# Jason9339/Wavelet-Noise-in-ray-tracing

Measured on AMD Instinct MI355X. Metric: Mnoise-samples/sec (3D wavelet, octave=4), higher is better.
Workload: dtype f32; 1 GPU; 512^3 dense 3D WNoise grid, tile=128, octave=4 (configs[1]); tile=128, seed=12345, octave=4, device=AMD Radeon Graphics (gfx950:sramecc+:xnack-)

## Files before the change

wavelet-noise-in-ray-tracing_amd/csrc/wn_api.hip:

```cpp
#include "wn_internal.hpp"

#include <algorithm>
#include <cstdlib>
#include <cstring>
#include <map>
#include <mutex>
#include <numeric>
#include <random>
#include <utility>
#include <vector>

namespace wn {

static char g_private_rand_state[256];
static std::mutex g_rand_mu;
static int g_rand_depth = 0;
static char *g_rand_caller = nullptr;

RandStateGuard::RandStateGuard()
{
    std::lock_guard<std::mutex> lock(g_rand_mu);
    if (g_rand_depth++ == 0) {
        static bool initialised = false;
        if (!initialised) {
// ... 295 lines not shown
    if (e != hipSuccess) {
        delete x;
        return hip_fail(e, "hipEventCreate");
    }
    *t = x;
    return WN_OK;
}
int wn_timer_start(wn_timer *t, void *stream)
{
    WN_ENTRY();
    if (!t) return fail(WN_ERR_INVALID, "timer is NULL");
    WN_HIP(hipEventRecord(t->start, as_stream(stream)));
    return WN_OK;
}
int wn_timer_stop(wn_timer *t, void *stream)
{
    WN_ENTRY();
    if (!t) return fail(WN_ERR_INVALID, "timer is NULL");
    WN_HIP(hipEventRecord(t->stop, as_stream(stream)));
    return WN_OK;
}
int wn_timer_elapsed_ms(wn_timer *t, float *ms)
{
    WN_ENTRY();
    if (!t || !ms) return fail(WN_ERR_INVALID, "timer/ms is NULL");
    WN_HIP(hipEventSynchronize(t->stop));
    WN_HIP(hipEventElapsedTime(ms, t->start, t->stop));
    return WN_OK;
}
void wn_timer_destroy(wn_timer *t)
{
    WN_ENTRY();
    if (!t) return;
    if (t->start) (void)hipEventDestroy(t->start);
    if (t->stop) (void)hipEventDestroy(t->stop);
    delete t;
}

int wn_gaussian_fill(uint32_t seed, size_t count, float *out_host)
{
    WN_ENTRY();
    if (count && !out_host) return fail(WN_ERR_INVALID, "out_host is NULL");
    std::mt19937 engine(seed);
    std::normal_distribution<float> gauss(0.0f, 1.0f);
    for (size_t i = 0; i < count; ++i) out_host[i] = gauss(engine);
    return WN_OK;
}

int wn_perlin_permutation(uint32_t seed, int out512_host[512])
{
    WN_ENTRY();
    if (!out512_host) return fail(WN_ERR_INVALID, "out512_host is NULL");
    std::vector<int> v(256);
    std::iota(v.begin(), v.end(), 0);
    std::shuffle(v.begin(), v.end(), std::mt19937(seed));
    for (int i = 0; i < 256; ++i) out512_host[i] = out512_host[i + 256] = v[i];
    return WN_OK;
}

int wn_tile_even_size(int requested) { return (requested % 2 != 0) ? requested + 1 : requested; }

static int tile_alloc(int n, int dims, wn_tile **out)
{
    if (!out) return fail(WN_ERR_INVALID, "out is NULL");
    *out = nullptr;
    if (dims != 2 && dims != 3) return fail(WN_ERR_INVALID, "dims must be 2 or 3 (got %d)", dims);
    if (n < 0) return fail(WN_ERR_INVALID, "tile size must be >= 0 (got %d)", n);
    if (n > 1024 || (dims == 3 && n > 1024)) return fail(WN_ERR_INVALID, "tile size %d too large", n);
    int rc = require_device();
    if (rc) return rc;
    wn_tile *t = new wn_tile();
    t->n = n;
    t->dims = dims;
    t->count = (dims == 2) ? (size_t)n * n : (size_t)n * n * n;
    (void)hipGetDevice(&t->device);
    if (t->count) {
        hipError_t e = hipMalloc(reinterpret_cast<void **>(&t->dev), t->count * sizeof(float));
        if (e != hipSuccess) {
            delete t;
            hip_fail(e, "hipMalloc(tile)");
            return WN_ERR_ALLOC;
        }
    }
    *out = t;
    return WN_OK;
}

int wn_tile_create(int n, int dims, const float *coeffs_host, wn_tile **out)
{
    WN_ENTRY();
    if (!coeffs_host) n = 0;
    if (n % 2 != 0)
        return fail(WN_ERR_INVALID, "wn_tile_create: coefficient tiles have even size (got %d)", n);
    int rc = tile_alloc(n, dims, out);
    if (rc) return rc;
    if ((*out)->count) {
        hipError_t e = hipMemcpy((*out)->dev, coeffs_host, (*out)->count * sizeof(float),
                                 hipMemcpyHostToDevice);
        if (e != hipSuccess) {
            wn_tile_destroy(*out);
            *out = nullptr;
            return hip_fail(e, "hipMemcpy(tile)");
        }
        rc = tile_build_padded(*out, nullptr);
        if (rc) {
            wn_tile_destroy(*out);
            *out = nullptr;
            return rc;
        }
    }
    return WN_OK;
}

int wn_tile_generate_from_field(int n, int dims, const float *field_host, wn_tile **out)
{
    WN_ENTRY();
    if (!field_host && n > 0) return fail(WN_ERR_INVALID, "field_host is NULL");
    if (n % 2 != 0) return fail(WN_ERR_INVALID, "tile size must be even (got %d)", n);
    int rc = tile_alloc(n, dims, out);
    if (rc) return rc;
    wn_tile *t = *out;
    if (!t->count) return WN_OK;
    float *field_dev = nullptr;
    hipError_t e = hipMalloc(reinterpret_cast<void **>(&field_dev), t->count * sizeof(float));
    if (e == hipSuccess)
        e = hipMemcpy(field_dev, field_host, t->count * sizeof(float), hipMemcpyHostToDevice);
    if (e != hipSuccess) {
        if (field_dev) (void)hipFree(field_dev);
        wn_tile_destroy(t);
        *out = nullptr;
        return hip_fail(e, "tile field upload");
    }
    rc = wn::tilegen_filter(t, field_dev, nullptr);
    hipError_t se = hipStreamSynchronize(nullptr);
    (void)hipFree(field_dev);
    if (rc == WN_OK && se != hipSuccess) rc = hip_fail(se, "tile generation");
    if (rc == WN_OK) rc = tile_build_padded(t, nullptr);
    if (rc) {
        wn_tile_destroy(t);
        *out = nullptr;
    }
    return rc;
}

int wn_tile_generate(int n, int dims, uint32_t seed, wn_tile **out)
{
    WN_ENTRY();
    if (n < 0) return fail(WN_ERR_INVALID, "tile size must be >= 0");
    if (dims != 2 && dims != 3) return fail(WN_ERR_INVALID, "dims must be 2 or 3 (got %d)", dims);
    const int even = wn_tile_even_size(n);
    if (even != n)
        fprintf(stderr, "Warning: Tile size adjusted to %d (must be even)\n", even);
    const size_t count = (dims == 2) ? (size_t)even * even : (size_t)even * even * even;
    std::vector<float> field(count);
    wn_gaussian_fill(seed, count, field.data());
    return wn_tile_generate_from_field(even, dims, field.data(), out);
}

int wn_tile_size(const wn_tile *t) { return t ? t->n : 0; }
int wn_tile_dims(const wn_tile *t) { return t ? t->dims : 0; }
size_t wn_tile_count(const wn_tile *t) { return t ? t->count : 0; }
const float *wn_tile_device_ptr(const wn_tile *t) { return t ? t->dev : nullptr; }

int wn_tile_download(const wn_tile *t, float *out_host)
{
    WN_ENTRY();
    if (!t) return fail(WN_ERR_INVALID, "tile is NULL");
    if (!t->count) return WN_OK;
    if (!out_host) return fail(WN_ERR_INVALID, "out_host is NULL");
    WN_HIP(hipMemcpy(out_host, t->dev, t->count * sizeof(float), hipMemcpyDeviceToHost));
    return WN_OK;
}

void wn_tile_destroy(wn_tile *t)
{
    WN_ENTRY();
    if (!t) return;
    if (t->dev) (void)hipFree(t->dev);
    if (t->dev_padded) (void)hipFree(t->dev_padded);
    delete t;
}

int wn_perm_create(const int table512_host[512], wn_perm **out)
{
    WN_ENTRY();
    if (!out) return fail(WN_ERR_INVALID, "out is NULL");
    *out = nullptr;
    if (!table512_host) return fail(WN_ERR_INVALID, "table is NULL");
    uint8_t bytes[512];
    for (int i = 0; i < 512; ++i) {
        if (table512_host[i] < 0 || table512_host[i] > 255)
            return fail(WN_ERR_INVALID, "permutation entry %d out of 0..255", i);
        bytes[i] = (uint8_t)table512_host[i];
    }
    int rc = require_device();
    if (rc) return rc;
    wn_perm *p = new wn_perm();
    std::memcpy(p->host, table512_host, sizeof(p->host));
    (void)hipGetDevice(&p->device);
    hipError_t e = hipMalloc(reinterpret_cast<void **>(&p->dev), 512);
    if (e == hipSuccess) e = hipMemcpy(p->dev, bytes, 512, hipMemcpyHostToDevice);
    if (e != hipSuccess) {
        if (p->dev) (void)hipFree(p->dev);
        delete p;
        return hip_fail(e, "perm upload");
    }
    *out = p;
    return WN_OK;
}

int wn_perm_create_seeded(uint32_t seed, wn_perm **out)
{
    WN_ENTRY();
    int table[512];
    wn_perlin_permutation(seed, table);
    return wn_perm_create(table, out);
}

int wn_perm_download(const wn_perm *p, int out512_host[512])
{
    WN_ENTRY();
    if (!p || !out512_host) return fail(WN_ERR_INVALID, "perm/out is NULL");
    uint8_t bytes[512];
    WN_HIP(hipMemcpy(bytes, p->dev, 512, hipMemcpyDeviceToHost));
    for (int i = 0; i < 512; ++i) out512_host[i] = bytes[i];
    return WN_OK;
}

void wn_perm_destroy(wn_perm *p)
{
    WN_ENTRY();
    if (!p) return;
    if (p->dev) (void)hipFree(p->dev);
    delete p;
}

}
```

wavelet-noise-in-ray-tracing_amd/csrc/wn_internal.hpp:

```cpp
#pragma once

#include <hip/hip_runtime.h>

#include <cmath>
#include <cstdarg>
#include <cstddef>
#include <cstdint>
#include <cstdio>

#include "wn_eval.hpp"
#include "wnoise.h"
#include "wnoise_advect.h"

typedef float v4f __attribute__((ext_vector_type(4)));

struct wn_tile {
    int n = 0;
    int dims = 0;
    size_t count = 0;
    float *dev = nullptr;
    float *dev_padded = nullptr;
    int device = 0;
};

struct wn_perm {
    int host[512];
    uint8_t *dev = nullptr;
    int device = 0;
};

struct wn_timer {
    hipEvent_t start = nullptr, stop = nullptr;
};

namespace wn {

void set_error(const char *fmt, ...);
int fail(int code, const char *fmt, ...);
int hip_fail(hipError_t e, const char *what);
int require_device();

inline hipStream_t as_stream(void *s) { return reinterpret_cast<hipStream_t>(s); }

class RandStateGuard {
  public:
    RandStateGuard();
    ~RandStateGuard();
    RandStateGuard(const RandStateGuard &) = delete;
    RandStateGuard &operator=(const RandStateGuard &) = delete;
};
#define WN_ENTRY() ::wn::RandStateGuard wn_rand_state_guard_

#define WN_HIP(call)                                            \
    do {                                                        \
        hipError_t _e = (call);                                 \
        if (_e != hipSuccess) return ::wn::hip_fail(_e, #call); \
    } while (0)

#define WN_LAUNCH_CHECK(name)                                    \
    do {                                                         \
        hipError_t _e = hipGetLastError();                       \
        if (_e != hipSuccess) return ::wn::hip_fail(_e, name);   \
    } while (0)

struct GridArgs {
    int den, nx, ny, z0, nz;
    float base_range, octave_scale, post_scale;
    int z_const_mode;
    float z_const;
    float out_scale;
};

int check_grid(const wn_grid *g, bool needs_z, GridArgs *out);

inline float inv_den_of(int den) { return ((den & (den - 1)) == 0) ? 1.0f / (float)den : 0.0f; }

int current_device();
int device_compute_units(int dev);
bool ensure_dynamic_lds(const void *kernel, int dev, size_t bytes);
int check_handle_device(int handle_device, const char *what);
int check_tile(const wn_tile *tile, int dims, const char *entry);
int check_perm(const wn_perm *perm, const char *entry);

inline bool vec4_ok(const float *out, int nx) { return nx % 4 == 0 && (reinterpret_cast<uintptr_t>(out) & 15) == 0; }

constexpr size_t kStrideBlockCap = 256u * 8u * 8u;
inline int stride_blocks(size_t total, size_t cap = kStrideBlockCap)
{
    const size_t b = (total + 255) / 256;
    return (int)(b < 1 ? 1 : (b > cap ? cap : b));
}

struct LatticeStep {
    double step;
    double pmax;
    double slack;
    long long extent(int samples) const { return (long long)floor((samples - 1) * step + slack) + 1 + 3; }
    bool two_mids() const { return 3.0 * step + slack <= 1.0; }
};

inline bool lattice_step(const GridArgs &g, float oscale, bool with_z_const, bool signed_step, double margin_cells,
                         LatticeStep *ls)
{
    double step = (double)g.base_range * (double)oscale * (double)g.post_scale / g.den;
// ... 148 lines not shown
```

wavelet-noise-in-ray-tracing_amd/csrc/wn_wavelet_multiband.hip:

```cpp
#include "wn_internal.hpp"

#include <algorithm>
#include <cmath>
#include <type_traits>

namespace {

using wn::GridArgs;

typedef float v4f __attribute__((ext_vector_type(4)));
typedef float v2f __attribute__((ext_vector_type(2)));

constexpr int kMaxNB = 5;
constexpr int kWW = 8, kPW = 4, kSW = 4;
constexpr int kWaves = kWW + kPW + kSW;
constexpr int kPasses = 2 * kPW;
constexpr int kBX = 512, kBY = 8, kBZ = 8;
constexpr int kRing = 4;
constexpr int kSlotZ = 8, kSlotX = 16;
constexpr int kMaxK = 5;
constexpr int kRRow = kPasses * 64;
constexpr int kRPlane = kBY * kRRow;
constexpr int kRingFloats = kRing * kBY * kBX;
constexpr int kBoxFloats = 6144;
constexpr int kDmaPlanes = kMaxNB;
constexpr int kDmaLanded = kBZ - 2;

struct MbBand {
    float oscale;
    float factor;
    int first_pass;
    int K;
    int box_off;
    int rowlen;
};

struct MbArgs {
    const float *coef;
    float *out;
    int n, nmask;
    GridArgs g;
    float inv_den;
    int nbx, nby, nbz;
    int all_full;
    MbBand band[kMaxNB];
    int pass_band[kPasses];
};

__device__ __forceinline__ float readlane_f(float v, int l)
{
    return __int_as_float(__builtin_amdgcn_readlane(__float_as_int(v), l));
}

template <int NB>
__global__ __launch_bounds__(64 * kWaves) void grid3d_mbp_kernel(const MbArgs a)
{
    extern __shared__ __attribute__((aligned(16))) float lds[];
    __shared__ __attribute__((aligned(16))) float s_box[kBoxFloats];
    __shared__ int s_mid[3][NB][32];
    __shared__ float s_w[3][NB][kSlotX][3];
    __shared__ float s_oscale[NB];
    __shared__ __attribute__((aligned(16))) float s_wy[NB][kMaxK][kBY];
    __shared__ float s_wz[NB][64];
    __shared__ int s_prep[NB][4];
    __shared__ int s_bandc[NB][4];

    const int tid = threadIdx.x, lane = tid & 63;
    const int wave = __builtin_amdgcn_readfirstlane(tid >> 6);
    const bool is_window = wave < kWW, is_collapse = wave >= kWW && wave < kWW + kPW;
    const GridArgs &g = a.g;
    float *const ring = lds + 2 * kRPlane;

    const int nyz = a.nby * a.nbz;
    const long long total = (long long)a.nbx * nyz;
    const int item0 = (int)(total * blockIdx.x / gridDim.x), item1 = (int)(total * (blockIdx.x + 1) / gridDim.x);
    const int nb = item1 - item0;
    if (nb <= 0) return;
    const int G = nb * kBZ;

    struct Brick { int bx, by, bz; };
    auto brick_of = [&](int item) {
        Brick k;
        k.bx = item / nyz;
        k.by = (item - k.bx * nyz) / a.nbz;
        k.bz = item - k.bx * nyz - k.by * a.nbz;
        return k;
    };
    auto advance = [&](Brick &k) {
        if (++k.bz == a.nbz) { k.bz = 0; ++k.by; }
        if (k.by == a.nby) { k.by = 0; ++k.bx; }
    };

    auto fill_tables = [&](int buf, const Brick &k) {
        int tt = tid;
        asm volatile("" : "+v"(tt));
        const int b = tt >> 5, slot = tt & 31;
        if (b < NB && slot < kSlotX + 2) {
            int idx;
            if (slot < kSlotZ) idx = min(k.by * kBY + slot, g.ny - 1);
            else if (slot < kSlotX) idx = g.z0 + min(k.bz * kBZ + slot - kSlotZ, g.nz - 1);
            else idx = (slot == kSlotX) ? k.bx * kBX : min(k.bx * kBX + kBX - 1, g.nx - 1);
            const float c = wn::lattice_coord_fast(idx, (float)g.den, a.inv_den, g.base_range, s_oscale[b], g.post_scale);
            int m;
            float w0, w1, w2;
            wn::bspline(c, m, w0, w1, w2);
            s_mid[buf][b][slot] = m;
            if (slot < kSlotX) {
                s_w[buf][b][slot][0] = w0;
                s_w[buf][b][slot][1] = w1;
                s_w[buf][b][slot][2] = w2;
            }
        }
    };
    auto sgpr = [](int v) { return __builtin_amdgcn_readfirstlane(v); };
    auto fresh_rows = [&](int b, int K, int tA, int tB, bool same_column) {
        const int d = sgpr(s_mid[tB][b][kSlotZ]) - sgpr(s_mid[tA][b][kSlotZ]);
        return (same_column && d >= 0 && d <= 2) ? d : K;
    };

    auto derive_tables = [&](int b, int tA, int tB, bool same_column, bool first) {
        const int l = lane;
        {
            const int K = s_bandc[b][0];
            const int kz0 = s_mid[tB][b][kSlotZ] - 1;
            const int kzm = (K == 4) ? (kz0 & 3) : ((kz0 + 20 * 65536) % 5);
            {
                const int zi = l >> 3, j = l & 7;
                int t0 = kzm + (s_mid[tB][b][kSlotZ + zi] - s_mid[tB][b][kSlotZ]);
                t0 -= (t0 >= K) ? K : 0;
                const float w0 = s_w[tB][b][kSlotZ + zi][0], w1 = s_w[tB][b][kSlotZ + zi][1], w2 = s_w[tB][b][kSlotZ + zi][2];
                s_wz[b][l] = j == 0 ? w0 : j == 1 ? w1 : j == 2 ? w2 : __int_as_float(t0);
            }
            if (l < kMaxK * kBY) {
                const int j = l >> 3, yi = l & 7;
                const int dd = j - (s_mid[tB][b][yi] - s_mid[tB][b][0]);
                const float w0 = s_w[tB][b][yi][0], w1 = s_w[tB][b][yi][1], w2 = s_w[tB][b][yi][2];
                float f = a.band[0].factor;
#pragma unroll
                for (int bb = 1; bb < NB; ++bb) f = (b == bb) ? a.band[bb].factor : f;
                s_wy[b][j][yi] = ((unsigned)dd <= 2u ? (dd == 0 ? w0 : dd == 1 ? w1 : w2) : 0.0f) * f;
            }
            if (l == 0) {
                const int dz = s_mid[tB][b][kSlotZ] - s_mid[tA][b][kSlotZ];
                s_prep[b][0] = kzm;
                s_prep[b][1] = (!first && same_column && dz >= 0 && dz <= 2) ? dz : K;
                s_prep[b][2] = (s_mid[tB][b][kSlotX] - 1) & 3;
            }
        }
    };

    Brick cur = brick_of(item0), nxt = cur;
    advance(nxt);
    Brick nxt2 = nxt;
    advance(nxt2);
    if (tid < NB) {
        int K = a.band[0].K, box_off = a.band[0].box_off, rowlen = a.band[0].rowlen, fp = a.band[0].first_pass;
#pragma unroll
        for (int bb = 1; bb < NB; ++bb) {
            K = (tid == bb) ? a.band[bb].K : K;
            box_off = (tid == bb) ? a.band[bb].box_off : box_off;
            rowlen = (tid == bb) ? a.band[bb].rowlen : rowlen;
            fp = (tid == bb) ? a.band[bb].first_pass : fp;
        }
        s_bandc[tid][0] = K;
        s_bandc[tid][1] = box_off;
        s_bandc[tid][2] = rowlen;
        s_bandc[tid][3] = fp;
        float os = a.band[0].oscale;
#pragma unroll
        for (int bb = 1; bb < NB; ++bb) os = (tid == bb) ? a.band[bb].oscale : os;
        s_oscale[tid] = os;
    }
    __syncthreads();
    fill_tables(0, cur);
    if (nb > 1) fill_tables(1, nxt);
    __syncthreads();
    int tb = 0, t = 0;
    auto next_brick = [&]() {
        cur = nxt;
        nxt = nxt2;
        advance(nxt2);
        tb = (tb == 2) ? 0 : tb + 1;
        ++t;
    };

// ... 48 lines not shown
        };
        auto p1_slice = [&](float *Rw, int zi, const auto &yc, float wzv, auto kc) {
            constexpr int K = decltype(kc)::value;
            if constexpr (K > 0) {
                const float w0 = readlane_f(wzv, zi * 8), w1 = readlane_f(wzv, zi * 8 + 1), w2 = readlane_f(wzv, zi * 8 + 2);
                const int t0 = __builtin_amdgcn_readlane(__float_as_int(wzv), zi * 8 + 3);
                auto taps = [&](auto tc) {
                    constexpr int T0 = decltype(tc)::value, T1 = (T0 + 1) % K, T2 = (T0 + 2) % K;
#pragma unroll
                    for (int p2 = 0; p2 < kBY / 2; ++p2) {
                        v2f v = v2f{w0, w0} * yc[p2][T0];
                        v = __builtin_elementwise_fma(v2f{w1, w1}, yc[p2][T1], v);
                        v = __builtin_elementwise_fma(v2f{w2, w2}, yc[p2][T2], v);
                        Rw[(2 * p2) * kRRow] = v.x;
                        Rw[(2 * p2 + 1) * kRRow] = v.y;
                    }
                };
                using std::integral_constant;
                if (t0 == 0) taps(integral_constant<int, 0>{});
                else if (t0 == 1) taps(integral_constant<int, 1>{});
                else if (t0 == 2) taps(integral_constant<int, 2>{});
                else if (t0 == 3 || K == 4) taps(integral_constant<int, 3>{});
                else taps(integral_constant<int, K - 1>{});
            }
        };
        auto collapse_role = [&](auto k0c, auto k1c) {
            constexpr int K0 = decltype(k0c)::value, K1 = decltype(k1c)::value;
            v2f yc0[kBY / 2][K0 > 0 ? K0 : 1], yc1[kBY / 2][K1 > 0 ? K1 : 1];
            float wzv0 = 0.0f, wzv1 = 0.0f;
            float *const Rw0 = lds + 64 * ps[0].id + lane, *const Rw1 = lds + 64 * ps[1].id + lane;
            wn::lds_barrier();
            prep_brick(ps[0], yc0, wzv0, k0c);
            prep_brick(ps[1], yc1, wzv1, k1c);
            p1_slice(Rw0, 0, yc0, wzv0, k0c);
            p1_slice(Rw1, 0, yc1, wzv1, k1c);
            wn::lds_barrier();
            for (int gp = 0; gp < G + 2; ++gp) {
                const int zi = gp & (kBZ - 1);
                if (gp < G) {
                    if (gp + 1 < G) {
                        if (zi == kBZ - 1) {
                            prep_brick(ps[0], yc0, wzv0, k0c);
                            prep_brick(ps[1], yc1, wzv1, k1c);
                        }
                        const int rs = ((gp + 1) & 1) * kRPlane;
                        p1_slice(Rw0 + rs, (gp + 1) & (kBZ - 1), yc0, wzv0, k0c);
                        p1_slice(Rw1 + rs, (gp + 1) & (kBZ - 1), yc1, wzv1, k1c);
                    }
                    if (zi == kBZ - 1) next_brick();
                }
                wn::lds_barrier();
            }
        };
        using std::integral_constant;
        const int k0 = pk[0], k1 = pk[1];
        if (k0 == 4 && k1 == 4) collapse_role(integral_constant<int, 4>{}, integral_constant<int, 4>{});
        else if (k0 == 4 && k1 == 5) collapse_role(integral_constant<int, 4>{}, integral_constant<int, 5>{});
        else if (k0 == 5 && k1 == 4) collapse_role(integral_constant<int, 5>{}, integral_constant<int, 4>{});
        else if (k0 == 5 && k1 == 5) collapse_role(integral_constant<int, 5>{}, integral_constant<int, 5>{});
        else if (k0 == 4) collapse_role(integral_constant<int, 4>{}, integral_constant<int, 0>{});
        else if (k0 == 5) collapse_role(integral_constant<int, 5>{}, integral_constant<int, 0>{});
        else collapse_role(integral_constant<int, 0>{}, integral_constant<int, 0>{});
    } else if (is_window) {
        const int xw = (wave >> 2) & 1, wr = wave & 3;
        float ww[NB][4][4];
        int wbase[NB];
        auto x_weights = [&](int tbuf, int bx) {
            const float den = (float)g.den;
            const int x0 = bx * kBX + xw * 256 + lane * 4;
            float xbase[4];
#pragma unroll
            for (int q = 0; q < 4; ++q) {
                const float xi = (float)min(x0 + q, g.nx - 1);
                xbase[q] = ((a.inv_den != 0.0f) ? xi * a.inv_den : xi / den) * g.base_range;
            }
#pragma unroll
            for (int b = 0; b < NB; ++b) {
                int m[4];
                float w[4][3];
#pragma unroll
                for (int q = 0; q < 4; ++q) {
                    float cc = xbase[q] * a.band[b].oscale;
                    cc = cc * g.post_scale;
                    wn::bspline(cc, m[q], w[q][0], w[q][1], w[q][2]);
                }
                wbase[b] = 64 * a.band[b].first_pass + m[0] - s_mid[tbuf][b][kSlotX];
#pragma unroll
                for (int q = 0; q < 4; ++q) {
                    const bool up = m[q] != m[0];
                    ww[b][q][0] = up ? 0.0f : w[q][0];
                    ww[b][q][1] = up ? w[q][0] : w[q][1];
                    ww[b][q][2] = up ? w[q][1] : w[q][2];
                    ww[b][q][3] = up ? w[q][2] : 0.0f;
                }
            }
        };
        auto phaseC = [&](int rslot, int ringslot) {
            float acc[2][4];
            const float *Rp = lds + rslot * kRPlane + wr * kRRow;
#pragma unroll
            for (int b = 0; b < NB; ++b) {
                float v[2][4];
#pragma unroll
                for (int h = 0; h < 2; ++h)
#pragma unroll
                    for (int i = 0; i < 4; ++i) v[h][i] = Rp[h * 4 * kRRow + wbase[b] + i];
#pragma unroll
                for (int h = 0; h < 2; ++h)
#pragma unroll
                    for (int q = 0; q < 4; ++q) {
                        float s = (b == 0) ? ww[b][q][0] * v[h][0] : __builtin_fmaf(ww[b][q][0], v[h][0], acc[h][q]);
                        s = __builtin_fmaf(ww[b][q][1], v[h][1], s);
                        s = __builtin_fmaf(ww[b][q][2], v[h][2], s);
                        s = __builtin_fmaf(ww[b][q][3], v[h][3], s);
                        acc[h][q] = s;
                    }
            }
#pragma unroll
            for (int h = 0; h < 2; ++h)
                *reinterpret_cast<v4f *>(ring + (ringslot * kBY + wr + 4 * h) * kBX + xw * 256 + lane * 4) =
                    v4f{acc[h][0], acc[h][1], acc[h][2], acc[h][3]};
        };

        x_weights(0, cur.bx);
        wn::lds_barrier();
        wn::lds_barrier();
        for (int gp = 0; gp < G + 2; ++gp) {
            const int zi = gp & (kBZ - 1);
            if (gp < G) {
                phaseC(gp & 1, gp & (kRing - 1));
                if (zi == kBZ - 1) {
                    const int tb1 = (tb == 2) ? 0 : tb + 1, tb2 = (tb1 == 2) ? 0 : tb1 + 1;
                    if (t + 2 < nb) fill_tables(tb2, nxt2);
                    if (t + 1 < nb && nxt.bx != cur.bx) x_weights(tb1, nxt.bx);
                    next_brick();
                }
            }
            wn::lds_barrier();
        }
    } else {
        const int sw = wave - (kWW + kPW);
        int bK[NB], bBox[NB], bRow[NB];
#pragma unroll
        for (int b = 0; b < NB; ++b) {
            bK[b] = sgpr(s_bandc[b][0]);
            bBox[b] = sgpr(s_bandc[b][1]);
            bRow[b] = sgpr(s_bandc[b][2]);
        }
        auto request_band = [&](auto bc, int tA, int tB, bool same_column, bool first) {
            constexpr int b = decltype(bc)::value;
            if constexpr (b < NB) {
                const int K = bK[b];
                const int d = first ? K : fresh_rows(b, K, tA, tB, same_column);
                const int jy0 = sgpr(s_mid[tB][b][0]) - 1, kz0 = sgpr(s_mid[tB][b][kSlotZ]) - 1 + (K - d);
                const int r = min(lane, K * K - 1);
                const int f = (K == 4) ? (r >> 2) : ((r * 13) >> 6);
                const int j = r - f * K;
                const int rowoff = (((kz0 + f) & a.nmask) * a.n + ((jy0 + j) & a.nmask)) * a.n;
                const int ix0 = (sgpr(s_mid[tB][b][kSlotX]) - 1) & ~3;
                const unsigned voff = (unsigned)((ix0 + 4 * lane) & a.nmask) * 4u;
                for (int rr = sw; rr < d * K; rr += kSW) {
                    const char *rowp = reinterpret_cast<const char *>(a.coef + __builtin_amdgcn_readlane(rowoff, rr));
                    if (4 * lane < bRow[b])
                        __builtin_amdgcn_global_load_lds((const __attribute__((address_space(1))) void *)(rowp + voff),
                                                         (__attribute__((address_space(3))) void *)&s_box[bBox[b] + rr * bRow[b]],
                                                         16, 0, 0);
                }
            }
        };
        Brick sb = cur;
        const size_t plane_stride = (size_t)g.ny * g.nx;
        float *orow = nullptr;
        auto brick_pointer = [&]() {
            orow = a.out + ((size_t)(sb.bz * kBZ) * g.ny + sb.by * kBY + 2 * sw) * g.nx + sb.bx * kBX + lane * 4;
        };
        brick_pointer();
        auto store_plane = [&](int p) {
            const int zi = p & (kBZ - 1), ringslot = p & (kRing - 1);
            const float *src = ring + (ringslot * kBY + 2 * sw) * kBX + lane * 4;
            v4f v[4];
#pragma unroll
            for (int q = 0; q < 4; ++q) v[q] = *reinterpret_cast<const v4f *>(src + (q >> 1) * kBX + (q & 1) * 256);
            if (a.all_full) {
#pragma unroll
                for (int q = 0; q < 4; ++q) *reinterpret_cast<v4f *>(orow + (size_t)(q >> 1) * g.nx + (q & 1) * 256) = v[q];
            } else {
                const int z = sb.bz * kBZ + zi;
#pragma unroll
                for (int q = 0; q < 4; ++q) {
                    const int row = 2 * sw + (q >> 1), xh = q & 1;
                    const int y = sb.by * kBY + row, x = sb.bx * kBX + xh * 256 + lane * 4;
                    if (y < g.ny && z < g.nz && x + 3 < g.nx)
                        *reinterpret_cast<v4f *>(orow + (size_t)(q >> 1) * g.nx + (q & 1) * 256) = v[q];
                }
            }
            orow += plane_stride;
            if (zi == kBZ - 1) {
                advance(sb);
                brick_pointer();
            }
        };

        using std::integral_constant;
        request_band(integral_constant<int, 0>{}, 0, 0, false, true);
        request_band(integral_constant<int, 1>{}, 0, 0, false, true);
        request_band(integral_constant<int, 2>{}, 0, 0, false, true);
        request_band(integral_constant<int, 3>{}, 0, 0, false, true);
        request_band(integral_constant<int, 4>{}, 0, 0, false, true);
        for (int b = sw; b < NB; b += kSW) derive_tables(b, 0, 0, false, true);
        asm volatile("s_waitcnt vmcnt(0)" ::: "memory");
        wn::lds_barrier();
        wn::lds_barrier();
        for (int gp = 0; gp < G + 2; ++gp) {
            const int zi = gp & (kBZ - 1);
            if (gp >= 2) store_plane(gp - 2);
            if (gp < G) {
                if (zi < NB && t + 1 < nb) {
                    const int tb1 = (tb == 2) ? 0 : tb + 1;
                    const bool same = nxt.bx == cur.bx && nxt.by == cur.by;
                    if (zi == 0) request_band(integral_constant<int, 0>{}, tb, tb1, same, false);
                    else if (zi == 1) request_band(integral_constant<int, 1>{}, tb, tb1, same, false);
                    else if (zi == 2) request_band(integral_constant<int, 2>{}, tb, tb1, same, false);
                    else if (zi == 3) request_band(integral_constant<int, 3>{}, tb, tb1, same, false);
                    else request_band(integral_constant<int, 4>{}, tb, tb1, same, false);
                }
                if (zi == kBZ - 2 && t + 1 < nb)
                    for (int b = sw; b < NB; b += kSW)
                        derive_tables(b, tb, (tb == 2) ? 0 : tb + 1, nxt.bx == cur.bx && nxt.by == cur.by, false);
                if (zi == kDmaLanded) {
                    if (a.all_full) asm volatile("s_waitcnt vmcnt(%0)" ::"n"(4 * (kDmaLanded - kDmaPlanes + 1)) : "memory");
                    else asm volatile("s_waitcnt vmcnt(0)" ::: "memory");
                }
                if (zi == kBZ - 1) next_brick();
            }
            wn::lds_barrier();
        }
    }
}

template <int NB>
bool launch_mbp(const MbArgs &a, size_t lds, long long bricks, hipStream_t s)
{
    const void *fn = reinterpret_cast<const void *>(&grid3d_mbp_kernel<NB>);
    if (!wn::ensure_dynamic_lds(fn, wn::current_device(), lds)) return false;
    const int cus = wn::device_compute_units(wn::current_device());
    const int grid = (int)std::min<long long>(bricks, cus);
    hipLaunchKernelGGL((grid3d_mbp_kernel<NB>), dim3(grid), dim3(64 * kWaves), lds, s, a);
    return true;
}

}

namespace wn {

int multiband_try(const wn_tile *tile, const GridArgs &g, int nbands, const float *oscale, const float *weights,
                  float out_div, float *out_dev, hipStream_t stream, int min_bricks_per_cu)
{
    if (nbands < 1 || nbands > kMaxNB || tile->n == 0 || wn::pow2_mask(tile->n) < 0) return kDeclined;
    if (g.nx <= 256 || !vec4_ok(out_dev, g.nx) || g.ny <= 0 || g.nz <= 0 || g.z_const_mode || g.z0 < 0) return kDeclined;
    MbArgs a{};
    int passes = 0, box_off = 0;
    for (int w = 0; w < kPasses; ++w) a.pass_band[w] = -1;
    for (int b = 0; b < nbands; ++b) {
        LatticeStep ls;
        if (!lattice_step(g, oscale[b], false, false, 0.0, &ls) || !ls.two_mids()) return kDeclined;
        const int K = (int)std::max<long long>(4, std::max(ls.extent(kBY), ls.extent(kBZ)));
        if (K > kMaxK) return kDeclined;
        const int ex = (int)ls.extent(kBX) + 1;
        const int np = (ex + 63) / 64;
        if (passes + np > kPasses) return kDeclined;
        a.band[b].first_pass = passes;
        for (int p = 0; p < np; ++p) a.pass_band[passes++] = b;
        a.band[b].oscale = oscale[b];
        a.band[b].factor = (float)((double)(weights ? weights[b] : 1.0f) * (double)g.out_scale / (double)out_div);
        a.band[b].K = K;
        a.band[b].rowlen = (ex + 3 + 3) & ~3;
        if (a.band[b].rowlen > 256) return kDeclined;
        a.band[b].box_off = box_off;
        box_off += K * K * a.band[b].rowlen;
    }
    if (box_off > kBoxFloats) return kDeclined;
    const size_t lds = (size_t)(2 * kRPlane + kRingFloats) * sizeof(float);
    a.coef = tile->dev;
    a.out = out_dev;
    a.n = tile->n;
    a.nmask = wn::pow2_mask(tile->n);
    a.g = g;
    a.inv_den = wn::inv_den_of(g.den);
    a.nbx = (g.nx + kBX - 1) / kBX;
    a.nby = (g.ny + kBY - 1) / kBY;
    a.nbz = (g.nz + kBZ - 1) / kBZ;
    a.all_full = (g.nx % kBX == 0 && g.ny % kBY == 0 && g.nz % kBZ == 0) ? 1 : 0;
    const long long bricks = (long long)a.nbx * a.nby * a.nbz;
    if (bricks > 0x7fffffffLL / kBZ) return kDeclined;
    if (bricks < (long long)min_bricks_per_cu * wn::device_compute_units(wn::current_device())) return kDeclined;
    if ((long long)a.nbx * kBX * 10 > (long long)g.nx * 11) return kDeclined;
    bool ok;
    switch (nbands) {
    case 1: ok = launch_mbp<1>(a, lds, bricks, stream); break;
    case 2: ok = launch_mbp<2>(a, lds, bricks, stream); break;
    case 3: ok = launch_mbp<3>(a, lds, bricks, stream); break;
    case 4: ok = launch_mbp<4>(a, lds, bricks, stream); break;
    default: ok = launch_mbp<5>(a, lds, bricks, stream); break;
    }
    if (!ok) return kDeclined;
    WN_LAUNCH_CHECK("grid3d_mbp_kernel");
    return WN_OK;
}

}
```

Before: 1.389 million Msamples/s.

## Merge lower octave bands into one pre-upsampled coefficient box before evaluation

For three or more bands whose scales double each step, a new prepass kernel algebraically folds all lower octaves into a single dense coefficient field sampled at the top band's lattice (half-cell shifted). It uses B-spline upsampling weights of 0.75/0.25 and writes the field to per-tile scratch. The main kernel then evaluates only two spline bands instead of NB, reading the merged box from scratch. The volume is processed in z-chunks sized to fit the scratch. The cost is an extra kernel launch per chunk, scratch memory traffic, and an event to order reuse of the scratch buffer.

Result: slower. 1.368 million Msamples/s (-1.5%).

```diff
diff --git a/wavelet-noise-in-ray-tracing_amd/csrc/wn_api.hip b/wavelet-noise-in-ray-tracing_amd/csrc/wn_api.hip
--- a/wavelet-noise-in-ray-tracing_amd/csrc/wn_api.hip
+++ b/wavelet-noise-in-ray-tracing_amd/csrc/wn_api.hip
@@ -401,6 +401,15 @@
             return WN_ERR_ALLOC;
         }
     }
+    if (t->count && dims == 3) {
+        hipError_t e = hipMalloc(reinterpret_cast<void **>(&t->merge_scratch), wn::kMergeScratchBytes);
+        if (e == hipSuccess) e = hipEventCreateWithFlags(&t->merge_done, hipEventDisableTiming);
+        if (e != hipSuccess) {
+            wn_tile_destroy(t);
+            hip_fail(e, "hipMalloc(tile scratch)");
+            return WN_ERR_ALLOC;
+        }
+    }
     *out = t;
     return WN_OK;
 }
@@ -497,6 +506,8 @@
     if (!t) return;
     if (t->dev) (void)hipFree(t->dev);
     if (t->dev_padded) (void)hipFree(t->dev_padded);
+    if (t->merge_scratch) (void)hipFree(t->merge_scratch);
+    if (t->merge_done) (void)hipEventDestroy(t->merge_done);
     delete t;
 }
 
diff --git a/wavelet-noise-in-ray-tracing_amd/csrc/wn_internal.hpp b/wavelet-noise-in-ray-tracing_amd/csrc/wn_internal.hpp
--- a/wavelet-noise-in-ray-tracing_amd/csrc/wn_internal.hpp
+++ b/wavelet-noise-in-ray-tracing_amd/csrc/wn_internal.hpp
@@ -9,6 +9,7 @@
 #include <cstdio>
 
 #include "wn_eval.hpp"
+#include "wn_merge_plan.hpp"
 #include "wnoise.h"
 #include "wnoise_advect.h"
 
@@ -20,6 +21,8 @@
     size_t count = 0;
     float *dev = nullptr;
     float *dev_padded = nullptr;
+    float *merge_scratch = nullptr;
+    hipEvent_t merge_done = nullptr;
     int device = 0;
 };
 
diff --git a/wavelet-noise-in-ray-tracing_amd/csrc/wn_merge_plan.hpp b/wavelet-noise-in-ray-tracing_amd/csrc/wn_merge_plan.hpp
--- /dev/null
+++ b/wavelet-noise-in-ray-tracing_amd/csrc/wn_merge_plan.hpp
@@ -0,0 +1,74 @@
+#pragma once
+
+#include <algorithm>
+#include <climits>
+#include <cmath>
+#include <cstddef>
+
+namespace wn {
+
+constexpr size_t kMergeScratchBytes = (size_t)16 << 20;
+constexpr int kMergeBrickX = 512, kMergeBrickYZ = 8;
+
+struct MergeRange {
+    long long lo, hi;
+    long long count() const { return hi - lo + 1; }
+};
+
+inline long long merge_mid_min(double step, double slack, long long i) { return (long long)ceil(i * step - 1.0 - slack); }
+inline long long merge_mid_max(double step, double slack, long long i) { return (long long)ceil(i * step - 1.0 + slack); }
+
+inline long long merge_floor4(long long v) { return v - (((v % 4) + 4) % 4); }
+
+inline MergeRange merge_rows(double step, double slack, long long i0, long long count, int K)
+{
+    const long long last = i0 + count - 1, last_brick = i0 + (count - 1) / kMergeBrickYZ * kMergeBrickYZ;
+    MergeRange r;
+    r.lo = merge_mid_min(step, slack, i0) - 1;
+    r.lo -= ((r.lo % 2) + 2) % 2;
+    r.hi = std::max(merge_mid_max(step, slack, last) + 1, merge_mid_max(step, slack, last_brick) - 1 + (K - 1));
+    return r;
+}
+
+inline MergeRange merge_columns(double step, double slack, long long nx, int rowlen)
+{
+    const long long last_brick = (nx - 1) / kMergeBrickX * kMergeBrickX;
+    MergeRange r;
+    r.lo = merge_floor4(merge_mid_min(step, slack, 0) - 1);
+    const long long end = std::max(merge_mid_max(step, slack, nx - 1) + 2, merge_floor4(merge_mid_max(step, slack, last_brick) - 1) + rowlen);
+    r.hi = r.lo + ((end - r.lo + 3) / 4) * 4 - 1;
+    return r;
+}
+
+inline long long merge_z_rows_bound(double step, double slack, long long planes, int K)
+{
+    const long long last_brick = (planes - 1) / kMergeBrickYZ * kMergeBrickYZ;
+    const long long by_last = (long long)floor((planes - 1) * step + 2.0 * slack) + 1 + 2;
+    const long long by_brick = (long long)floor(last_brick * step + 2.0 * slack) + 1 + (K - 1);
+    return std::max(by_last, by_brick) + 1 + 1;
+}
+
+struct MergePlan {
+    MergeRange x, y;
+    long long z_rows;
+    long long chunk_planes;
+};
+
+inline bool merge_plan(double step, double slack, int nx, int ny, int K, int rowlen, size_t capacity, MergePlan *p)
+{
+    if (nx <= 0 || ny <= 0 || !(step >= 0.0)) return false;
+    p->x = merge_columns(step, slack, nx, rowlen);
+    p->y = merge_rows(step, slack, 0, ny, K);
+    const long long footprint = p->x.count() * p->y.count();
+    if (footprint <= 0 || (unsigned long long)footprint > capacity) return false;
+    p->z_rows = (long long)(capacity / (unsigned long long)footprint);
+    if (merge_z_rows_bound(step, slack, kMergeBrickYZ, K) > p->z_rows) return false;
+    long long planes = (long long)(INT_MAX / kMergeBrickYZ) * kMergeBrickYZ;
+    if (step > 0.0 && (double)p->z_rows / step < (double)planes - 2 * kMergeBrickYZ)
+        planes = (long long)((double)p->z_rows / step) / kMergeBrickYZ * kMergeBrickYZ + kMergeBrickYZ;
+    while (planes > kMergeBrickYZ && merge_z_rows_bound(step, slack, planes, K) > p->z_rows) planes -= kMergeBrickYZ;
+    p->chunk_planes = planes;
+    return true;
+}
+
+}
diff --git a/wavelet-noise-in-ray-tracing_amd/csrc/wn_wavelet_multiband.hip b/wavelet-noise-in-ray-tracing_amd/csrc/wn_wavelet_multiband.hip
--- a/wavelet-noise-in-ray-tracing_amd/csrc/wn_wavelet_multiband.hip
+++ b/wavelet-noise-in-ray-tracing_amd/csrc/wn_wavelet_multiband.hip
@@ -23,6 +23,9 @@
 constexpr int kRPlane = kBY * kRRow;
 constexpr int kRingFloats = kRing * kBY * kBX;
 constexpr int kBoxFloats = 6144;
+constexpr int kBoxFloatsMerged = 8192;
+constexpr int kMergeFrom = 3;
+constexpr int box_floats(int nb) { return nb >= kMergeFrom ? kBoxFloatsMerged : kBoxFloats; }
 constexpr int kDmaPlanes = kMaxNB;
 constexpr int kDmaLanded = kBZ - 2;
 
@@ -45,18 +48,25 @@
     int all_full;
     MbBand band[kMaxNB];
     int pass_band[kPasses];
+    const float *msrc;
+    int m_ox, m_oy, m_oz, m_sx, m_sy, m_sz;
 };
+
+template <int NB>
+constexpr bool from_merged_box(int b) { return NB >= kMergeFrom && b == 0; }
 
 __device__ __forceinline__ float readlane_f(float v, int l)
 {
     return __int_as_float(__builtin_amdgcn_readlane(__float_as_int(v), l));
 }
 
-template <int NB>
+template <int NBANDS>
 __global__ __launch_bounds__(64 * kWaves) void grid3d_mbp_kernel(const MbArgs a)
 {
+    constexpr bool kMerged = NBANDS >= kMergeFrom;
+    constexpr int NB = kMerged ? 2 : NBANDS;
     extern __shared__ __attribute__((aligned(16))) float lds[];
-    __shared__ __attribute__((aligned(16))) float s_box[kBoxFloats];
+    __shared__ __attribute__((aligned(16))) float s_box[box_floats(NBANDS)];
     __shared__ int s_mid[3][NB][32];
     __shared__ float s_w[3][NB][kSlotX][3];
     __shared__ float s_oscale[NB];
@@ -100,7 +110,8 @@
             if (slot < kSlotZ) idx = min(k.by * kBY + slot, g.ny - 1);
             else if (slot < kSlotX) idx = g.z0 + min(k.bz * kBZ + slot - kSlotZ, g.nz - 1);
             else idx = (slot == kSlotX) ? k.bx * kBX : min(k.bx * kBX + kBX - 1, g.nx - 1);
-            const float c = wn::lattice_coord_fast(idx, (float)g.den, a.inv_den, g.base_range, s_oscale[b], g.post_scale);
+            float c = wn::lattice_coord_fast(idx, (float)g.den, a.inv_den, g.base_range, s_oscale[b], g.post_scale);
+            if constexpr (kMerged) c = (b == 0) ? c - 0.5f : c;
             int m;
             float w0, w1, w2;
             wn::bspline(c, m, w0, w1, w2);
@@ -315,6 +326,7 @@
                 for (int q = 0; q < 4; ++q) {
                     float cc = xbase[q] * a.band[b].oscale;
                     cc = cc * g.post_scale;
+                    if constexpr (kMerged) cc = (b == 0) ? cc - 0.5f : cc;
                     wn::bspline(cc, m[q], w[q][0], w[q][1], w[q][2]);
                 }
                 wbase[b] = 64 * a.band[b].first_pass + m[0] - s_mid[tbuf][b][kSlotX];
@@ -389,11 +401,22 @@
                 const int r = min(lane, K * K - 1);
                 const int f = (K == 4) ? (r >> 2) : ((r * 13) >> 6);
                 const int j = r - f * K;
-                const int rowoff = (((kz0 + f) & a.nmask) * a.n + ((jy0 + j) & a.nmask)) * a.n;
                 const int ix0 = (sgpr(s_mid[tB][b][kSlotX]) - 1) & ~3;
-                const unsigned voff = (unsigned)((ix0 + 4 * lane) & a.nmask) * 4u;
+                int rowoff;
+                unsigned voff;
+                const float *src;
+                if constexpr (from_merged_box<NBANDS>(b)) {
+                    const int kr = min(max(kz0 + f - a.m_oz, 0), a.m_sz - 1), jr = min(max(jy0 + j - a.m_oy, 0), a.m_sy - 1);
+                    rowoff = (kr * a.m_sy + jr) * a.m_sx + min(max(ix0 - a.m_ox, 0), a.m_sx - bRow[b]);
+                    voff = (unsigned)(4 * lane) * 4u;
+                    src = a.msrc;
+                } else {
+                    rowoff = (((kz0 + f) & a.nmask) * a.n + ((jy0 + j) & a.nmask)) * a.n;
+                    voff = (unsigned)((ix0 + 4 * lane) & a.nmask) * 4u;
+                    src = a.coef;
+                }
                 for (int rr = sw; rr < d * K; rr += kSW) {
-                    const char *rowp = reinterpret_cast<const char *>(a.coef + __builtin_amdgcn_readlane(rowoff, rr));
+                    const char *rowp = reinterpret_cast<const char *>(src + __builtin_amdgcn_readlane(rowoff, rr));
                     if (4 * lane < bRow[b])
                         __builtin_amdgcn_global_load_lds((const __attribute__((address_space(1))) void *)(rowp + voff),
                                                          (__attribute__((address_space(3))) void *)&s_box[bBox[b] + rr * bRow[b]],
@@ -471,6 +494,189 @@
     }
 }
 
+constexpr int kMgX = 32, kMgY = 8, kMgZ = 8;
+constexpr int kMgLds = 7 * 7 * 18;
+constexpr int kMgC = 6 * 6 * 17;
+
+struct MergeArgs {
+    const float *coef;
+    float *M;
+    int n, nmask;
+    int ox, oy, oz, sx, sy, sz;
+    float factor[kMaxNB - 1];
+};
+
+struct MgRegion {
+    const float *p;
+    int x0, y0, z0, nx, ny;
+};
+
+template <bool FIRST>
+__device__ __forceinline__ float merge_value(float f, int hx, int hy, int hz, const MgRegion &c, const MgRegion &prev)
+{
+    const int ex = hx & 1, ey = hy & 1, ez = hz & 1;
+    const int mx = hx >> 1, my = hy >> 1, mz = hz >> 1;
+    const float wx[2] = {ex ? 0.25f : 0.75f, ex ? 0.75f : 0.25f}, wy[2] = {ey ? 0.25f : 0.75f, ey ? 0.75f : 0.25f},
+                wz[2] = {ez ? 0.25f : 0.75f, ez ? 0.75f : 0.25f};
+    float w[2][2][2];
+#pragma unroll
+    for (int dz = 0; dz < 2; ++dz)
+#pragma unroll
+        for (int dy = 0; dy < 2; ++dy)
+#pragma unroll
+            for (int dx = 0; dx < 2; ++dx) w[dz][dy][dx] = (wz[dz] * wy[dy]) * wx[dx];
+    const float *cp = c.p + ((mz - c.z0) * c.ny + (my - c.y0)) * c.nx + (mx - c.x0);
+    float cs = 0.0f;
+#pragma unroll
+    for (int dz = 0; dz < 2; ++dz)
+#pragma unroll
+        for (int dy = 0; dy < 2; ++dy)
+#pragma unroll
+            for (int dx = 0; dx < 2; ++dx) {
+                const float v = cp[(dz * c.ny + dy) * c.nx + dx];
+                cs = (dz + dy + dx == 0) ? w[dz][dy][dx] * v : __builtin_fmaf(w[dz][dy][dx], v, cs);
+            }
+    if constexpr (FIRST) {
+        return f * cs;
+    } else {
+        const float *p = prev.p + ((mz - 1 + ez - prev.z0) * prev.ny + (my - 1 + ey - prev.y0)) * prev.nx + (mx - 1 + ex - prev.x0);
+        float hs = 0.0f;
+#pragma unroll
+        for (int dz = 0; dz < 2; ++dz)
+#pragma unroll
+            for (int dy = 0; dy < 2; ++dy)
+#pragma unroll
+                for (int dx = 0; dx < 2; ++dx) {
+                    const float v = p[(dz * prev.ny + dy) * prev.nx + dx];
+                    hs = (dz + dy + dx == 0) ? w[1 - dz][1 - dy][1 - dx] * v : __builtin_fmaf(w[1 - dz][1 - dy][1 - dx], v, hs);
+                }
+        return __builtin_fmaf(f, cs, hs);
+    }
+}
+
+__device__ __forceinline__ int mg_div(int e, int inv) { return (e * inv) >> 18; }
+__device__ __forceinline__ int mg_inv(int d) { return ((1 << 18) + d - 1) / d; }
+
+__device__ __forceinline__ void merge_group(float f, const float (&cv)[2][2][2], const float (&qv)[3][3][3], float (&out)[2][2][2])
+{
+#pragma unroll
+    for (int oz = 0; oz < 2; ++oz)
+#pragma unroll
+        for (int oy = 0; oy < 2; ++oy)
+#pragma unroll
+            for (int ox = 0; ox < 2; ++ox) {
+                float cs = 0.0f, hs = 0.0f;
+#pragma unroll
+                for (int dz = 0; dz < 2; ++dz)
+#pragma unroll
+                    for (int dy = 0; dy < 2; ++dy)
+#pragma unroll
+                        for (int dx = 0; dx < 2; ++dx) {
+                            const float wd = ((dz == oz ? 0.75f : 0.25f) * (dy == oy ? 0.75f : 0.25f)) * (dx == ox ? 0.75f : 0.25f);
+                            const float we = ((dz != oz ? 0.75f : 0.25f) * (dy != oy ? 0.75f : 0.25f)) * (dx != ox ? 0.75f : 0.25f);
+                            const float q = qv[oz + dz][oy + dy][ox + dx];
+                            cs = (dz + dy + dx == 0) ? wd * cv[dz][dy][dx] : __builtin_fmaf(wd, cv[dz][dy][dx], cs);
+                            hs = (dz + dy + dx == 0) ? we * q : __builtin_fmaf(we, q, hs);
+                        }
+                out[oz][oy][ox] = __builtin_fmaf(f, cs, hs);
+            }
+}
+
+template <int L>
+__global__ __launch_bounds__(256) void band_merge_kernel(const MergeArgs a)
+{
+    static_assert(L >= 2 && L < kMaxNB, "the bands below the top one of 3..5");
+    __shared__ float s_lvl[2][kMgLds];
+    __shared__ float s_c[L][kMgC];
+    const int tid = threadIdx.x;
+    int lo[L + 1][3], len[L + 1][3];
+    lo[L][0] = a.ox + kMgX * blockIdx.x, len[L][0] = min(kMgX, a.sx - kMgX * (int)blockIdx.x);
+    lo[L][1] = a.oy + kMgY * blockIdx.y, len[L][1] = min(kMgY, a.sy - kMgY * (int)blockIdx.y);
+    lo[L][2] = a.oz + kMgZ * blockIdx.z, len[L][2] = min(kMgZ, a.sz - kMgZ * (int)blockIdx.z);
+#pragma unroll
+    for (int l = L - 1; l >= 1; --l)
+#pragma unroll
+        for (int d = 0; d < 3; ++d) {
+            lo[l][d] = (lo[l + 1][d] >> 1) - 1;
+            len[l][d] = ((lo[l + 1][d] + len[l + 1][d] - 1) >> 1) + 1 - lo[l][d] + 1;
+        }
+    MgRegion c[L + 1];
+    int ccount[L + 1];
+    float cval[L + 1][2];
+    int cix[L + 1], ciy[L + 1];
+    auto c_index = [&](int l, int e) {
+        const int r = mg_div(e, cix[l]), x = e - r * c[l].nx, z = mg_div(r, ciy[l]), y = r - z * c[l].ny;
+        return (((c[l].z0 + z) & a.nmask) * a.n + ((c[l].y0 + y) & a.nmask)) * a.n + ((c[l].x0 + x) & a.nmask);
+    };
+#pragma unroll
+    for (int l = 1; l <= L; ++l) {
+        c[l] = MgRegion{s_c[l - 1], lo[l][0] >> 1, lo[l][1] >> 1, lo[l][2] >> 1, 0, 0};
+        c[l].nx = ((lo[l][0] + len[l][0] - 1) >> 1) + 2 - c[l].x0;
+        c[l].ny = ((lo[l][1] + len[l][1] - 1) >> 1) + 2 - c[l].y0;
+        ccount[l] = c[l].nx * c[l].ny * (((lo[l][2] + len[l][2] - 1) >> 1) + 2 - c[l].z0);
+        cix[l] = mg_inv(c[l].nx), ciy[l] = mg_inv(c[l].ny);
+#pragma unroll
+        for (int k = 0; k < 2; ++k) cval[l][k] = (tid + 256 * k < ccount[l]) ? a.coef[c_index(l, tid + 256 * k)] : 0.0f;
+    }
+#pragma unroll
+    for (int l = 1; l <= L; ++l) {
+#pragma unroll
+        for (int k = 0; k < 2; ++k)
+            if (tid + 256 * k < ccount[l]) s_c[l - 1][tid + 256 * k] = cval[l][k];
+        for (int e = tid + 512; e < ccount[l]; e += 256) s_c[l - 1][e] = a.coef[c_index(l, e)];
+    }
+    __syncthreads();
+#pragma unroll
+    for (int l = 1; l < L; ++l) {
+        const MgRegion prev{s_lvl[(l - 1) & 1], lo[l > 1 ? l - 1 : 1][0], lo[l > 1 ? l - 1 : 1][1], lo[l > 1 ? l - 1 : 1][2],
+                            len[l > 1 ? l - 1 : 1][0], len[l > 1 ? l - 1 : 1][1]};
+        float *cur = s_lvl[l & 1];
+        const int ix = mg_inv(len[l][0]), iy = mg_inv(len[l][1]);
+        for (int e = tid; e < len[l][0] * len[l][1] * len[l][2]; e += 256) {
+            const int r = mg_div(e, ix), x = e - r * len[l][0], z = mg_div(r, iy), y = r - z * len[l][1];
+            const int hx = lo[l][0] + x, hy = lo[l][1] + y, hz = lo[l][2] + z;
+            cur[e] = (l == 1) ? merge_value<true>(a.factor[0], hx, hy, hz, c[l], prev) : merge_value<false>(a.factor[l - 1], hx, hy, hz, c[l], prev);
+        }
+        __syncthreads();
+    }
+    const int gx = tid & 15, gy = (tid >> 4) & 3, gz = tid >> 6;
+    if (2 * gx < len[L][0] && 2 * gy < len[L][1] && 2 * gz < len[L][2]) {
+        const MgRegion &cc = c[L];
+        const MgRegion prev{s_lvl[(L - 1) & 1], lo[L - 1][0], lo[L - 1][1], lo[L - 1][2], len[L - 1][0], len[L - 1][1]};
+        const int jx = (lo[L][0] >> 1) + gx, jy = (lo[L][1] >> 1) + gy, jz = (lo[L][2] >> 1) + gz;
+        float cv[2][2][2], qv[3][3][3], out[2][2][2];
+        const float *cp = cc.p + ((jz - cc.z0) * cc.ny + (jy - cc.y0)) * cc.nx + (jx - cc.x0);
+        const float *qp = prev.p + ((jz - 1 - prev.z0) * prev.ny + (jy - 1 - prev.y0)) * prev.nx + (jx - 1 - prev.x0);
+#pragma unroll
+        for (int dz = 0; dz < 2; ++dz)
+#pragma unroll
+            for (int dy = 0; dy < 2; ++dy)
+#pragma unroll
+                for (int dx = 0; dx < 2; ++dx) cv[dz][dy][dx] = cp[(dz * cc.ny + dy) * cc.nx + dx];
+#pragma unroll
+        for (int dz = 0; dz < 3; ++dz)
+#pragma unroll
+            for (int dy = 0; dy < 3; ++dy)
+#pragma unroll
+                for (int dx = 0; dx < 3; ++dx) qv[dz][dy][dx] = qp[(dz * prev.ny + dy) * prev.nx + dx];
+        merge_group(a.factor[L - 1], cv, qv, out);
+        float *o = a.M + ((size_t)(kMgZ * blockIdx.z + 2 * gz) * a.sy + (kMgY * blockIdx.y + 2 * gy)) * a.sx + (kMgX * blockIdx.x + 2 * gx);
+#pragma unroll
+        for (int oz = 0; oz < 2; ++oz)
+#pragma unroll
+            for (int oy = 0; oy < 2; ++oy)
+                if (2 * gz + oz < len[L][2] && 2 * gy + oy < len[L][1])
+                    *reinterpret_cast<v2f *>(o + ((size_t)oz * a.sy + oy) * a.sx) = v2f{out[oz][oy][0], out[oz][oy][1]};
+    }
+}
+
+template <int L>
+void launch_merge(const MergeArgs &a, hipStream_t s)
+{
+    const dim3 grid((a.sx + kMgX - 1) / kMgX, (a.sy + kMgY - 1) / kMgY, (a.sz + kMgZ - 1) / kMgZ);
+    hipLaunchKernelGGL((band_merge_kernel<L>), grid, dim3(256), 0, s, a);
+}
+
 template <int NB>
 bool launch_mbp(const MbArgs &a, size_t lds, long long bricks, hipStream_t s)
 {
@@ -494,25 +700,53 @@
     MbArgs a{};
     int passes = 0, box_off = 0;
     for (int w = 0; w < kPasses; ++w) a.pass_band[w] = -1;
-    for (int b = 0; b < nbands; ++b) {
-        LatticeStep ls;
-        if (!lattice_step(g, oscale[b], false, false, 0.0, &ls) || !ls.two_mids()) return kDeclined;
-        const int K = (int)std::max<long long>(4, std::max(ls.extent(kBY), ls.extent(kBZ)));
-        if (K > kMaxK) return kDeclined;
-        const int ex = (int)ls.extent(kBX) + 1;
+    auto plan_spline = [&](int s, float os, float factor, LatticeStep *ls) {
+        if (!lattice_step(g, os, false, false, 0.0, ls) || !ls->two_mids()) return false;
+        const int K = (int)std::max<long long>(4, std::max(ls->extent(kBY), ls->extent(kBZ)));
+        if (K > kMaxK) return false;
+        const int ex = (int)ls->extent(kBX) + 1;
         const int np = (ex + 63) / 64;
-        if (passes + np > kPasses) return kDeclined;
-        a.band[b].first_pass = passes;
-        for (int p = 0; p < np; ++p) a.pass_band[passes++] = b;
-        a.band[b].oscale = oscale[b];
-        a.band[b].factor = (float)((double)(weights ? weights[b] : 1.0f) * (double)g.out_scale / (double)out_div);
-        a.band[b].K = K;
-        a.band[b].rowlen = (ex + 3 + 3) & ~3;
-        if (a.band[b].rowlen > 256) return kDeclined;
-        a.band[b].box_off = box_off;
-        box_off += K * K * a.band[b].rowlen;
-    }
+        if (passes + np > kPasses) return false;
+        a.band[s].first_pass = passes;
+        for (int p = 0; p < np; ++p) a.pass_band[passes++] = s;
+        a.band[s].oscale = os;
+        a.band[s].factor = factor;
+        a.band[s].K = K;
+        a.band[s].rowlen = (ex + 3 + 3) & ~3;
+        if (a.band[s].rowlen > 256) return false;
+        a.band[s].box_off = box_off;
+        box_off += K * K * a.band[s].rowlen;
+        return true;
+    };
+    auto factor_of = [&](int b) { return (float)((double)(weights ? weights[b] : 1.0f) * (double)g.out_scale / (double)out_div); };
+    const bool merged = nbands >= kMergeFrom;
+    LatticeStep ls{};
+    MergePlan mp{};
+    MergeArgs m{};
+    for (int b = 0; b < nbands; ++b)
+        if (!plan_spline(b, oscale[b], factor_of(b), &ls)) return kDeclined;
     if (box_off > kBoxFloats) return kDeclined;
+    if (merged) {
+        passes = box_off = 0;
+        for (int w = 0; w < kPasses; ++w) a.pass_band[w] = -1;
+        for (int b = 0; b < kMaxNB; ++b) a.band[b] = MbBand{};
+        const int top = nbands - 1;
+        for (int b = 0; b < top; ++b)
+            if (oscale[b + 1] != 2.0f * oscale[b]) return kDeclined;
+        if (!tile->merge_scratch) return kDeclined;
+        if (!plan_spline(0, oscale[top], 1.0f, &ls) || !plan_spline(1, oscale[top], factor_of(top), &ls)) return kDeclined;
+        if (!merge_plan(ls.step, ls.slack, g.nx, g.ny, a.band[0].K, a.band[0].rowlen, kMergeScratchBytes / sizeof(float), &mp))
+            return kDeclined;
+        if (mp.x.lo < INT_MIN / 2 || mp.y.lo < INT_MIN / 2) return kDeclined;
+        m.coef = tile->dev;
+        m.M = tile->merge_scratch;
+        m.n = tile->n;
+        m.nmask = wn::pow2_mask(tile->n);
+        m.ox = (int)mp.x.lo, m.sx = (int)mp.x.count();
+        m.oy = (int)mp.y.lo, m.sy = (int)mp.y.count();
+        for (int b = 0; b < top; ++b) m.factor[b] = factor_of(b);
+    }
+    if (box_off > box_floats(nbands)) return kDeclined;
     const size_t lds = (size_t)(2 * kRPlane + kRingFloats) * sizeof(float);
     a.coef = tile->dev;
     a.out = out_dev;
@@ -528,16 +762,49 @@
     if (bricks > 0x7fffffffLL / kBZ) return kDeclined;
     if (bricks < (long long)min_bricks_per_cu * wn::device_compute_units(wn::current_device())) return kDeclined;
     if ((long long)a.nbx * kBX * 10 > (long long)g.nx * 11) return kDeclined;
-    bool ok;
-    switch (nbands) {
-    case 1: ok = launch_mbp<1>(a, lds, bricks, stream); break;
-    case 2: ok = launch_mbp<2>(a, lds, bricks, stream); break;
-    case 3: ok = launch_mbp<3>(a, lds, bricks, stream); break;
-    case 4: ok = launch_mbp<4>(a, lds, bricks, stream); break;
-    default: ok = launch_mbp<5>(a, lds, bricks, stream); break;
-    }
-    if (!ok) return kDeclined;
-    WN_LAUNCH_CHECK("grid3d_mbp_kernel");
+    if (!merged) {
+        const bool ok = nbands == 1 ? launch_mbp<1>(a, lds, bricks, stream) : launch_mbp<2>(a, lds, bricks, stream);
+        if (!ok) return kDeclined;
+        WN_LAUNCH_CHECK("grid3d_mbp_kernel");
+        return WN_OK;
+    }
+    const void *fn = nbands == 3   ? reinterpret_cast<const void *>(&grid3d_mbp_kernel<3>)
+                     : nbands == 4 ? reinterpret_cast<const void *>(&grid3d_mbp_kernel<4>)
+                                   : reinterpret_cast<const void *>(&grid3d_mbp_kernel<5>);
+    if (!wn::ensure_dynamic_lds(fn, wn::current_device(), lds)) return kDeclined;
+    hipStreamCaptureStatus capture = hipStreamCaptureStatusNone;
+    if (hipStreamIsCapturing(stream, &capture) != hipSuccess) capture = hipStreamCaptureStatusNone;
+    const bool ordered = capture == hipStreamCaptureStatusNone && tile->merge_done;
+    if (ordered) WN_HIP(hipStreamWaitEvent(stream, tile->merge_done, 0));
+    a.msrc = m.M;
+    a.m_ox = m.ox, a.m_oy = m.oy, a.m_sx = m.sx, a.m_sy = m.sy;
+    for (long long c0 = 0; c0 < g.nz; c0 += mp.chunk_planes) {
+        const int planes = (int)std::min<long long>(mp.chunk_planes, g.nz - c0);
+        const MergeRange zr = merge_rows(ls.step, ls.slack, (long long)g.z0 + c0, planes, a.band[0].K);
+        if (zr.count() > mp.z_rows || zr.lo < INT_MIN / 2 || zr.hi > INT_MAX / 2)
+            return fail(WN_ERR_INVALID, "multiband grid: the merged box of planes %lld.. does not fit its plan", (long long)g.z0 + c0);
+        m.oz = (int)zr.lo, m.sz = (int)zr.count();
+        switch (nbands) {
+        case 3: launch_merge<2>(m, stream); break;
+        case 4: launch_merge<3>(m, stream); break;
+        default: launch_merge<4>(m, stream); break;
+        }
+        WN_LAUNCH_CHECK("band_merge_kernel");
+        a.g.z0 = g.z0 + (int)c0;
+        a.g.nz = planes;
+        a.out = out_dev + (size_t)c0 * g.ny * g.nx;
+        a.nbz = (planes + kBZ - 1) / kBZ;
+        a.all_full = (g.nx % kBX == 0 && g.ny % kBY == 0 && planes % kBZ == 0) ? 1 : 0;
+        a.m_oz = m.oz, a.m_sz = m.sz;
+        const long long chunk_bricks = (long long)a.nbx * a.nby * a.nbz;
+        switch (nbands) {
+        case 3: launch_mbp<3>(a, lds, chunk_bricks, stream); break;
+        case 4: launch_mbp<4>(a, lds, chunk_bricks, stream); break;
+        default: launch_mbp<5>(a, lds, chunk_bricks, stream); break;
+        }
+        WN_LAUNCH_CHECK("grid3d_mbp_kernel");
+    }
+    if (ordered) WN_HIP(hipEventRecord(tile->merge_done, stream));
     return WN_OK;
 }
 
```
